# aehogan/lammps-induced-dipole-polarization-pair-style

Measured on AMD Instinct MI355X. Metric: atom-steps/sec, higher is better.
Workload: dtype f64

## Files before the change

### include/polar_mi355x.h

```cpp
#ifndef POLAR_MI355X_H
#define POLAR_MI355X_H

#ifdef __cplusplus
extern "C" {
#endif

#define POLAR_OK 0
#define POLAR_WARN_NOT_CONVERGED 1
#define POLAR_RETRY_STEP 2
#define POLAR_ERR_INPUT -1
#define POLAR_ERR_NO_DEVICE -2
#define POLAR_ERR_HIP -3
#define POLAR_ERR_UNSUPPORTED -4
#define POLAR_ERR_STATE -5

enum { POLAR_DAMP_EXPONENTIAL = 0, POLAR_DAMP_NONE = 1 };

typedef struct polar_handle polar_handle;

typedef struct {
  double cut_lj_global, cut_coul;
  double polar_precision, polar_damp, polar_gamma;
  int iterations_max, damping_type, zodid, fixed_iteration;
  int polar_gs, polar_gs_ranked, use_previous, debug;
// ... 80 lines not shown
                  polar_result *out);
int polar_compute_peratom(polar_handle *h, int eflag, int vflag, double *f, double *mu, double *ef_static,
                          double *eatom, double *vatom, polar_result *out);

int polar_get_debug_trace(polar_handle *h, double *u_polar, int max);

int polar_get_debug_forces(polar_handle *h, double *out6);

int polar_get_colors(polar_handle *h, int *color, int n);

int polar_set_colors(polar_handle *h, const int *color, int n);

int polar_compute_resident(polar_handle *h, int eflag, int vflag, polar_result *out);
void *polar_dev_ptr(polar_handle *h, const char *name);
int polar_download(polar_handle *h, const char *name, double *dst, long long n);
int polar_upload_mu(polar_handle *h, const double *mu, long long n);


int polar_set_stream(polar_handle *h, void *hip_stream);
int polar_set_row_range(polar_handle *h, int lo, int hi);
int polar_set_global_count(polar_handle *h, long long natoms);
int polar_set_list_style(polar_handle *h, int full);
int polar_step_begin(polar_handle *h, int eflag, int vflag);
int polar_step_sweep(polar_handle *h);
int polar_step_sweep_phase(polar_handle *h, int color, int part);
int polar_step_sweep_part(polar_handle *h, int part, int nparts);
int polar_step_sweep_end(polar_handle *h, const double *dev_global_change);
int polar_step_sweep_end_n(polar_handle *h, const double *dev_global_change, int count);
int polar_step_state(polar_handle *h, int *done, int *iterations, int *status);
int polar_step_finish(polar_handle *h, polar_result *out);
// ... 36 lines not shown
```

### lammps-induced-dipole-polarization-pair-style_amd/__init__.py

```python
from __future__ import annotations

import ctypes as C
import importlib
import os
import subprocess

import numpy as np

_HERE = os.path.dirname(os.path.abspath(__file__))
_CSRC = os.path.join(_HERE, "csrc")
LIB_PATH = os.path.join(_HERE, "libpolar_mi355x.so")
LIB_PATH_LAB = os.path.join(_HERE, "libpolar_mi355x_lab.so")
HIPCC = os.environ.get("HIPCC", "/opt/rocm/bin/hipcc")
HIP_FLAGS = ["--offload-arch=gfx950", "-O3", "-std=c++17", "-fPIC", "-shared"]

_lib = None
_lib_lab = None


class PolarError(RuntimeError):

    def __init__(self, code, message):
        super().__init__(message)
        self.code = code
# ... 82 lines not shown
    "polar_set_settings": (C.c_int, [C.c_void_p, C.POINTER(Settings)]),
    "polar_set_types": (C.c_int, [C.c_void_p, C.c_int] + [_dp] * 7),
    "polar_set_coul": (C.c_int, [C.c_void_p, C.c_double, C.c_double, _dp, _dp, C.c_int, C.c_int, C.c_int, C.c_double]
                       + [_dp] * 8),
    "polar_set_box": (C.c_int, [C.c_void_p, _dp, _dp, _dp, _ip, C.c_int]),
    "polar_set_atoms": (C.c_int, [C.c_void_p, C.c_int, C.c_int, _dp, _dp, _dp, _ip, _ip]),
    "polar_set_positions": (C.c_int, [C.c_void_p, C.c_int, C.c_int, _dp]),
    "polar_set_neighbors": (C.c_int, [C.c_void_p, C.c_int, _ip, _ip, C.POINTER(_ip)]),
    "polar_set_neighbors_csr": (C.c_int, [C.c_void_p, C.c_int, _ip, _ip, _llp, _ip]),
    "polar_build_neighbors": (C.c_int, [C.c_void_p, _dp, _ip, _ip, _ip, C.c_int, _ip, C.c_int]),
    "polar_compute": (C.c_int, [C.c_void_p, C.c_int, C.c_int, _dp, _dp, _dp, C.POINTER(Result)]),
    "polar_compute_peratom": (C.c_int, [C.c_void_p, C.c_int, C.c_int, _dp, _dp, _dp, _dp, _dp, C.POINTER(Result)]),
    "polar_compute_resident": (C.c_int, [C.c_void_p, C.c_int, C.c_int, C.POINTER(Result)]),
    "polar_dev_ptr": (C.c_void_p, [C.c_void_p, C.c_char_p]),
    "polar_download": (C.c_int, [C.c_void_p, C.c_char_p, _dp, C.c_longlong]),
    "polar_upload_mu": (C.c_int, [C.c_void_p, _dp, C.c_longlong]),
    "polar_set_stream": (C.c_int, [C.c_void_p, C.c_void_p]),
    "polar_set_row_range": (C.c_int, [C.c_void_p, C.c_int, C.c_int]),
    "polar_set_global_count": (C.c_int, [C.c_void_p, C.c_longlong]),
    "polar_step_mu_get": (C.c_int, [C.c_void_p, C.c_longlong, C.c_longlong, _dp]),
    "polar_step_mu_put_idx": (C.c_int, [C.c_void_p, C.c_longlong, _ip, _dp]),
    "polar_step_change_get": (C.c_int, [C.c_void_p, _dp]),
    "polar_step_sweep_end_host": (C.c_int, [C.c_void_p, C.c_double]),
    "polar_step_sweep_end_n": (C.c_int, [C.c_void_p, C.c_void_p, C.c_int]),
    "polar_set_list_style": (C.c_int, [C.c_void_p, C.c_int]),
    "polar_set_newton": (C.c_int, [C.c_void_p, C.c_int]),
    "polar_get_debug_trace": (C.c_int, [C.c_void_p, _dp, C.c_int]),
    "polar_get_debug_forces": (C.c_int, [C.c_void_p, _dp]),
    "polar_get_colors": (C.c_int, [C.c_void_p, C.POINTER(C.c_int), C.c_int]),
    "polar_restart_pack": (C.c_int, [C.c_void_p, C.c_void_p, C.c_int]),
# ... 313 lines not shown
    def debug_forces(self):
        a = np.zeros(6)
        self._ck(self.L.polar_get_debug_forces(self.h, _dptr(a)))
        return a[:3].copy(), a[3:].copy()

    def colors(self, n):
        a = np.full(n, -1, dtype=np.int32)
        nc = self._ck(self.L.polar_get_colors(self.h, a.ctypes.data_as(C.POINTER(C.c_int)), n))
        return nc, a

    def download(self, name, n):
        a = np.zeros(n)
        self._ck(self.L.polar_download(self.h, name.encode(), _dptr(a), n))
        return a


class PolarDist:

    @staticmethod
    def unique_id():
        buf = C.create_string_buffer(128)
        rc = lib().polar_dist_unique_id(buf)
        if rc < 0:
            raise PolarError(rc, "polar_dist_unique_id failed (is RCCL available?)")
        return buf.raw

    def __init__(self, unique_id, rank, nranks, device=0):
        self.L = lib()
        self.d = C.c_void_p()
        self.rank, self.nranks = rank, nranks
# ... 101 lines not shown
```

### lammps-induced-dipole-polarization-pair-style_amd/csrc/polar_api.hip

```cpp
#include "polar_handle.hpp"

namespace {
void upload_types(polar_handle *h, int ntypes, const double *const t[7]) {
  need_device(h);
  const size_t m = (size_t)(ntypes + 1) * (ntypes + 1);
  std::vector<double> pack(8 * m, 0.0);
  for (size_t k = 0; k < m; k++) {
    pack[8 * k + 0] = t[6][k]; pack[8 * k + 1] = t[5][k]; pack[8 * k + 2] = t[0][k]; pack[8 * k + 3] = t[1][k];
    pack[8 * k + 4] = t[2][k]; pack[8 * k + 5] = t[3][k]; pack[8 * k + 6] = t[4][k];
  }
  h->d_lj.ensure(8 * m);
  HIPCHECK(hipMemcpy(h->d_lj.p, pack.data(), 8 * m * sizeof(double), hipMemcpyHostToDevice));
  h->P.ntypes = ntypes;
  h->P.ljpack = h->d_lj.p;
  h->ntypes = ntypes;
  h->types_set = true;
}

void upload_coul(polar_handle *h, double g_ewald, double qqrd2e, const double *slj, const double *scoul, int nbits,
                 int mask, int shift, double tabinnersq, const double *const t[8]) {
  need_device(h);
  h->P.g_ewald = g_ewald; h->P.qqrd2e = qqrd2e;
  for (int k = 0; k < 4; k++) { h->P.special_lj[k] = slj[k]; h->P.special_coul[k] = scoul[k]; }
  h->P.ncoultablebits = nbits; h->P.ncoulmask = mask; h->P.ncoulshiftbits = shift; h->P.tabinnersq = tabinnersq;
// ... 123 lines not shown
int polar_device_count(void) {
  int n = 0;
  if (hipGetDeviceCount(&n) != hipSuccess) return 0;
  return n;
}

int polar_create(int device, polar_handle **out) {
  if (!out) return POLAR_ERR_STATE;
  polar_handle *h = new polar_handle();
  *out = h;
  h->device = device;
  if (const char *e = getenv("POLAR_COLOR_DIST")) h->color_dist = atof(e);
  h->color_keep = std::max(h->color_dist - 0.4, 0.75 * h->color_dist);
  if (const char *e = getenv("POLAR_COLOR_KEEP")) h->color_keep = atof(e);
  if (const char *e = getenv("POLAR_DETERMINISTIC")) h->deterministic = atoi(e) != 0;
#ifdef POLAR_LAB
#include "lab/api_env_knobs.inc"
#endif
  int n = polar_device_count();
  if (n <= 0 || device < 0 || device >= n) {
    h->have_device = false;
    h->err = "no usable HIP device";
    return POLAR_OK;
  }
  return guarded(h, [&]() {
    HIPCHECK(hipSetDevice(device));
    HIPCHECK(hipStreamCreate(&h->stream));
    for (auto &e : h->ev) HIPCHECK(hipEventCreate(&e));
    {
      int prio_lo = 0, prio_hi = 0;
// ... 37 lines not shown
    for (hipEvent_t e : h->ev_nl) (void)hipEventDestroy(e);
    for (hipEvent_t e : h->ev_fchunk) if (e) (void)hipEventDestroy(e);
    h->d_ljpos.release(); h->d_ljaux.release(); h->d_tag.release(); h->d_nspecial.release(); h->d_special.release();
    h->d_ljcell_id.release(); h->d_ljcell_cnt.release(); h->d_ljcell_fill.release(); h->d_ljcell_first.release(); h->d_cutneighsq.release();
    h->d_xchg.release(); h->d_xidx.release();
    h->d_eatom.release(); h->d_vatom.release(); h->d_dd_r2.release(); h->d_fpol.release();
    h->d_x.release(); h->d_q.release(); h->d_alpha.release(); h->d_f.release(); h->d_ef.release(); h->d_F.release();
    h->d_mu.release(); h->d_mu0.release(); h->d_acc_x.release(); h->d_acc_f.release(); h->d_acc_g.release(); h->d_acc_dF.release(); h->d_acc_dG.release(); h->d_acc_part.release(); h->d_acc_state.release(); h->d_bflag.release(); h->d_rank.release(); h->d_dmu.release(); h->d_tab.release(); h->d_lj.release();
    h->d_type.release(); h->d_mol.release(); h->d_order.release(); h->d_pos.release(); h->d_ilist.release();
    h->d_numneigh.release(); h->d_neigh.release(); h->d_rows.release(); h->d_first.release();
    h->d_sym_first.release(); h->d_sym_cnt.release(); h->d_sym_fill.release(); h->d_sym_j.release();
    h->d_mol_s.release(); h->d_perm.release(); h->d_inv.release(); h->d_rows_orig.release(); h->d_ownrows.release(); h->d_ef_s.release(); h->d_scan_a.release(); h->d_scan_b.release(); h->d_gs_cnt.release(); h->d_T6.release(); h->d_Minv.release(); h->d_gsN.release(); h->d_gsAT.release(); h->d_cb.release(); h->d_gs_part.release();
    h->d_rec0.release(); h->d_rec1.release(); h->d_scal.release(); h->d_slots.release();
    h->d_cell_id.release(); h->d_cell_cnt.release(); h->d_cell_fill.release();
    h->d_nl_cnt.release(); h->d_dd_cnt.release(); h->d_dd_wrap.release(); h->d_lpdesc.release(); h->d_slot.release(); h->d_color_orig.release(); h->d_color_s.release(); h->d_trace.release(); h->d_ew_kv.release(); h->d_ew_hkl.release(); h->d_ew_rows.release(); h->d_ew_s.release(); h->d_ew_m.release(); h->d_ew_part.release(); h->d_ew_erec.release(); h->d_ew_vpart.release(); h->d_ew_out.release(); h->d_cl_orig.release(); h->d_cl_cnt.release(); h->d_cl_wrap.release(); h->d_cl_tw.release(); h->d_cl_s.release(); h->d_nl_j.release(); h->d_dd_j.release();
    h->d_cell_first.release(); h->d_nl_first.release(); h->d_dd_first.release(); h->d_dd_s.release(); h->d_xq.release(); h->d_pos4.release();
    h->d_overflow.release(); h->d_ddtot.release();
    h->d_cadj.release(); h->d_cdeg.release(); h->d_ccnt.release(); h->d_cflags.release(); h->d_crelabel.release(); h->d_klist.release(); h->d_dbgf.release(); h->d_ulead.release(); h->d_udd_j.release(); h->d_upos.release(); h->d_unit.release(); h->d_udesc.release(); h->d_cprio.release(); h->d_cstat.release(); h->d_coff.release(); h->d_lp_pend.release(); h->d_lp_part.release();
    if (h->h_cflags) (void)hipHostFree(h->h_cflags);
    if (h->h_cstat) (void)hipHostFree(h->h_cstat);
    if (h->h_coff) (void)hipHostFree(h->h_coff);
    h->d_srec0.release(); h->d_srec1.release(); h->d_thdr.release(); h->d_trow.release(); h->d_un_j.release(); h->d_dd16.release(); h->d_pend.release();
    if (h->h_flags) (void)hipHostFree(h->h_flags);
    if (h->h_ddtot) (void)hipHostFree(h->h_ddtot);
    if (h->h_scal) (void)hipHostFree(h->h_scal);
    if (h->h_stage) (void)hipHostFree(h->h_stage);
    for (auto &e : h->ev) if (e) (void)hipEventDestroy(e);
    if (h->stream && h->own_stream) (void)hipStreamDestroy(h->stream);
  }
  delete h;
  return POLAR_OK;
// ... 474 lines not shown
    if (!out) throw std::runtime_error("polar_compute_resident: null result pointer");
    need_device(h);
    HIPCHECK(hipSetDevice(h->device));
    return do_compute(h, eflag, vflag, nullptr, out);
  });
}

void *polar_dev_ptr(polar_handle *h, const char *name) {
  if (!h || !name || !h->have_device) return nullptr;
  if (strcmp(name, "f") == 0) return h->d_f.p;
  if (strcmp(name, "mu") == 0) return h->d_mu.p;
  if (strcmp(name, "ef_static") == 0) return h->d_ef.p;
  if (strcmp(name, "x") == 0) return h->d_x.p;
  if (strcmp(name, "eatom") == 0) return h->d_eatom.p;
  if (strcmp(name, "vatom") == 0) return h->d_vatom.p;
  return nullptr;
}
int polar_download(polar_handle *h, const char *name, double *dst, long long n) {
  return guarded(h, [&]() {
    need_device(h);
    void *p = polar_dev_ptr(h, name);
    if (!p) throw std::runtime_error("polar_download: unknown array name");
    HIPCHECK(hipMemcpy(dst, p, (size_t)n * sizeof(double), hipMemcpyDeviceToHost));
    return POLAR_OK;
  });
}
int polar_upload_mu(polar_handle *h, const double *mu, long long n) {
  return guarded(h, [&]() {
    need_device(h);
    h->d_mu.ensure((size_t)n);
    HIPCHECK(hipMemcpy(h->d_mu.p, mu, (size_t)n * sizeof(double), hipMemcpyHostToDevice));
// ... 278 lines not shown
```

### lammps-induced-dipole-polarization-pair-style_amd/csrc/polar_handle.hpp

```cpp
#pragma once
#include <hip/hip_runtime.h>

#include <algorithm>
#include <initializer_list>
#include <utility>
#include <chrono>
#include <cmath>
#include <cstdio>
#include <cstdlib>
#include <exception>
#include <cstring>
#include <numeric>
#include <string>
#include <thread>
#include <mutex>
#include <condition_variable>
#include <functional>
#include <memory>
#include <stdexcept>
#include <unistd.h>
#include <vector>

#include "pair_host.hpp"
#include "polar_kernels.hpp"

using namespace polar;

#define POLAR_KERNEL_VERSION "r05-lp3-v3"
#define POLAR_MAX_CLASS_OFF 130


struct HipError : std::runtime_error {
  explicit HipError(const std::string &m) : std::runtime_error(m) {}
};
struct NoDevice : std::runtime_error {
  NoDevice() : std::runtime_error("no usable HIP device: this library has no CPU fallback") {}
};
#define HIPCHECK(expr)                                                                             \
  do {                                                                                             \
    hipError_t e_ = (expr);                                                                        \
    if (e_ != hipSuccess)                                                                          \
      throw HipError(std::string(#expr) + " failed: " + hipGetErrorString(e_) + " (" + __FILE__ + \
                     ":" + std::to_string(__LINE__) + ")");                                      \
// ... 98 lines not shown
  DBuf<double2> d_dd_s;
  DBuf<int2> d_lpdesc;
  DBuf<double> d_lp_pend;
  DBuf<double> d_lp_part;
  int lp_npart = 0;
  DBuf<int> d_slot;
  std::vector<int> h_cl;
  DBuf<int> d_cl_orig, d_cl_cnt, d_cl_wrap, d_cl_tw;
  DBuf<int4> d_cl_s;
  long long cl_pitch = 0;
  int ncl = 0;
  double cluster_dist = 2.0;
  int cluster_max = 4;
  long long cl_slots = 0;
  DBuf<double4> d_xq, d_pos4, d_xq_s;
  long long nl_pairs = 0, dd_pairs = 0;
  long long nl_pitch = 0, dd_pitch = 0;
  DBuf<int> d_overflow;
  DBuf<unsigned long long> d_ddtot;
  int *h_flags = nullptr;
  unsigned long long *h_ddtot = nullptr;
  int inum = 0;
  long long nneigh = 0;
  bool mu_resident = false;
  DBuf<double> d_dbgf;
  DBuf<double> d_acc_x, d_acc_f, d_acc_g, d_acc_dF, d_acc_dG, d_acc_part;
  DBuf<AccelState> d_acc_state;
  long long acc_pitch = 0; int acc_rows = 0;
  DBuf<double> d_mu0;
  bool mu0_saved = false;
// ... 82 lines not shown
  TileLaunch tile_all{};
  size_t tile_lds_attr[16] = {0, 0, 0, 0, 0, 0, 0, 0, 0, 0, 0, 0, 0, 0, 0, 0};
  size_t tile_build_lds_attr = 0;
  int tile_waves = 4;
  int tile_wide = 0;
  int tile_sw[3] = {2, 2, 2};
  int deterministic = 0;
  Scal *h_scal = nullptr;
  hipEvent_t ev[8] = {};
  hipStream_t lj_stream = nullptr;
  hipEvent_t ev_fork = nullptr, ev_join = nullptr, ev_lj0 = nullptr, ev_lj1 = nullptr, ev_dl0 = nullptr, ev_dl1 = nullptr;
  hipStream_t dl_stream = nullptr;
  hipEvent_t ev_mu_ready = nullptr;
  double *early_mu = nullptr, *early_ef = nullptr, *user_mu = nullptr, *user_ef = nullptr;
  hipEvent_t ev_fchunk[4] = {nullptr, nullptr, nullptr, nullptr};
  bool overlap_lj = true;
  bool lj_forked = false;
  std::vector<double> h_tmp;
  double *h_stage = nullptr;
  DBuf<double> d_trace;
  DBuf<double4> d_ew_kv; DBuf<int4> d_ew_hkl, d_ew_rows;
  DBuf<double2> d_ew_s, d_ew_m, d_ew_part;
  DBuf<double> d_ew_erec, d_ew_vpart, d_ew_out;
  std::vector<double> ew_key;
  int ew_nk = 0, ew_nrow = 0, ew_nm = 0;
  double ew_cell[6] = {0, 0, 0, 0, 0, 0};
  hipEvent_t ev_ks[4] = {nullptr, nullptr, nullptr, nullptr};
  int ntrace = 0;
  size_t h_stage_cap = 0;
};
// ... 188 lines not shown
```

### lammps-induced-dipole-polarization-pair-style_amd/csrc/polar_lists.hpp

```cpp
#pragma once

#include "polar_common.hpp"

namespace polar {

struct CellGrid {
  int trim;
  int nc[3];
  double lo[3], inv[3];
};

__device__ __forceinline__ int cell_of(const CellGrid &g, const Box &b, double x, double y, double z) {
  int c[3];
  double fr3[3];
  frac_coords(b, g.lo, x, y, z, fr3);
#pragma unroll
  for (int k = 0; k < 3; k++) {
    double fr = fr3[k];
    fr -= floor(fr);
    int ck = (int)(fr * g.nc[k]);
    c[k] = ck >= g.nc[k] ? g.nc[k] - 1 : ck;
  }
  return (c[2] * g.nc[1] + c[1]) * g.nc[0] + c[0];
}
// ... 543 lines not shown
          if (RECHECK && icol >= 0 && rsq < colordistsq && __double2loint(rj.w) && color_s[j] == icol) clash = true;
          wrap_lane |= in_dd && shifted;
          same = (imol != 0 && imol == __double2hiint(rj.w)) ? POLAR_NL_SAMEMOL : 0;
        }
        const unsigned long long m_nl = __ballot(in_nl), m_dd = __ballot(in_dd);
        const int kn = ncount + __popcll(m_nl & below), kd = dcount + __popcll(m_dd & below);
        if (in_nl && kn < nl_pitch) nl_j[nl0 + kn] = j | same;
        if (in_dd && kd < dd_pitch) {
          dd_j[dd0 + (dd_shift ? lp_slot(kd, dd_qm) : (long long)kd)] = j << dd_shift;
          if (dd_r2) dd_r2[dd0 + kd] = rsq;
        }
        ncount += __popcll(m_nl);
        dcount += __popcll(m_dd);
      }
    }
  }
  if (pad_dd) {
    const int have = dcount < dd_pitch ? dcount : (int)dd_pitch;
    const int padded = (have + 63) & ~63;
    for (int k = have + lane; k < padded; k += 64) {
      dd_j[dd0 + (dd_shift ? lp_slot(k, dd_qm) : (long long)k)] = (dd_pad_index >= 0 ? dd_pad_index : i) << dd_shift;
      if (dd_r2) dd_r2[dd0 + k] = 1e60;
    }
  }
  if (RECHECK && color_s && __ballot(clash) != 0ull && lane == 0) atomicOr(color_conflict, 1);
  const unsigned long long anywrap = __ballot(wrap_lane);
  if (lane == 0) {
    nl_cnt[i] = ncount; dd_cnt[i] = dcount;
    if (dd_wrap) dd_wrap[i] = anywrap != 0ull;
    if (ncount > nl_pitch || dcount > dd_pitch) atomicMax(overflow, ncount > dcount ? ncount : dcount);
// ... 252 lines not shown
```

### lammps-induced-dipole-polarization-pair-style_amd/csrc/polar_rows.hpp

```cpp
#pragma once

#include "polar_common.hpp"

namespace polar {

static __global__ void k_pack(int n, const int *__restrict__ perm, const double *__restrict__ x, const double *__restrict__ q,
                       const double *__restrict__ alpha, const int *__restrict__ mol, const double *__restrict__ mu0,
                       AtomRec *__restrict__ r0, AtomRec *__restrict__ r1, int *__restrict__ mol_s,
                       double4 *__restrict__ pos4, double4 *__restrict__ xq_s, int wrap, Box box, double lo0, double lo1,
                       double lo2) {
  int i = blockIdx.x * blockDim.x + threadIdx.x;
  if (i == n) {
    AtomRec d;
    d.x = n > 0 ? x[0] : 0.0; d.y = n > 0 ? x[1] : 0.0; d.z = n > 0 ? x[2] : 0.0;
    d.mx = d.my = d.mz = d.q = d.a = 0.0;
    r0[n] = d; r1[n] = d;
  }
  if (i >= n) return;
  const int o = perm ? perm[i] : i;
  AtomRec r;
  r.x = x[3 * o]; r.y = x[3 * o + 1]; r.z = x[3 * o + 2]; r.q = q[o];
  if (wrap) {
    const double lo[3] = {lo0, lo1, lo2};
    double fr[3];
    frac_coords(box, lo, r.x, r.y, r.z, fr);
    const double n2 = box.periodic[2] ? floor(fr[2]) : 0.0, n1 = box.periodic[1] ? floor(fr[1]) : 0.0,
                 n0 = box.periodic[0] ? floor(fr[0]) : 0.0;
    r.z -= n2 * box.prd[2]; r.y -= n2 * box.yz + n1 * box.prd[1]; r.x -= n2 * box.xz + n1 * box.xy + n0 * box.prd[0];
  }
  r.mx = mu0 ? mu0[3 * o] : 0.0; r.my = mu0 ? mu0[3 * o + 1] : 0.0; r.mz = mu0 ? mu0[3 * o + 2] : 0.0;
  r.a = alpha[o];
  r0[i] = r;
  r1[i] = r;
  mol_s[i] = mol[o];
  if (pos4) pos4[i] = make_double4(r.x, r.y, r.z, __hiloint2double(mol[o], r.a != 0.0 ? 1 : 0));
  if (xq_s) xq_s[i] = make_double4(r.x, r.y, r.z, r.q);
}

template <bool ALLPAIRS, int PASS>
static __global__ __launch_bounds__(POLAR_BLOCK) void k_rank(int nlocal, int ntotal, const double *__restrict__ x,
                                                      const double *__restrict__ alpha, const int *__restrict__ mol,
                                                      Box box, RowList nl,
                                                      const int *__restrict__ nl_j,
                                                      const AtomRec *__restrict__ rec,
                                                      const int *__restrict__ mol_s, Scal *scal,
                                                      double *__restrict__ slots,
                                                      double *__restrict__ rank_metric, int nchunk) {
  const int lane = threadIdx.x & 63;
  const int gw = blockIdx.x * POLAR_ROWS_PER_BLOCK + (threadIdx.x >> 6);
  if (gw >= nlocal * nchunk) return;
  const int i = gw % nlocal, chunk = gw / nlocal;
// ... 614 lines not shown
```

### lammps-induced-dipole-polarization-pair-style_amd/csrc/polar_step.hip

```cpp
#include "polar_handle.hpp"

void launch_scan(long long n, const int *in, long long *out, DBuf<long long> &tot, hipStream_t s) {
  const int nb = (int)std::max<long long>(1, (n + POLAR_SCAN_ITEMS - 1) / POLAR_SCAN_ITEMS);
  tot.ensure((size_t)nb + 1);
  k_scan_block<<<nb, 1024, 0, s>>>(n, in, out, tot.p);
  if (nb > 1) {
    k_scan_totals<<<1, 1024, 0, s>>>(nb, tot.p, out + n);
    k_scan_add<<<nblk(n - POLAR_SCAN_ITEMS, 256), 256, 0, s>>>(n, out, tot.p);
  }
}

void build_cells(polar_handle *h) {
  const polar_settings &st = h->ph.st;
  const int n = h->nlocal;
  const double cutall = std::max(st.cut_coul, st.dd_cutoff);
  double width[3];
  box_widths(h->box, width);
  for (int k = 0; k < 3; k++)
    if (h->box.periodic[k] && width[k] < 2.0 * cutall * (1.0 - 1e-12))
      throw InputError("dd_cutoff mode needs box lengths >= 2*max(cut_coul,dd_cutoff); use exact mode (dd_cutoff 0)");
  CellGrid &g = h->grid;
  g.trim = 1;
#ifdef POLAR_LAB
  if (const char *e = getenv("POLAR_NL_TRIM")) g.trim = atoi(e);
// ... 23 lines not shown
    }
    h->tile_launches.clear();
    for (const Cls &cz : cls[2]) for (const Cls &cy : cls[1]) for (const Cls &cx : cls[0]) {
      TileLaunch L;
      L.start[0] = cx.start; L.stride[0] = cx.stride; L.count[0] = cx.count;
      L.start[1] = cy.start; L.stride[1] = cy.stride; L.count[1] = cy.count;
      L.start[2] = cz.start; L.stride[2] = cz.stride; L.count[2] = cz.count;
      for (int k = 0; k < 3; k++) L.nc[k] = g.nc[k];
      h->tile_launches.push_back(L);
    }
    for (int k = 0; k < 3; k++) { h->tile_all.start[k] = 0; h->tile_all.stride[k] = 1; h->tile_all.count[k] = g.nc[k]; h->tile_all.nc[k] = g.nc[k]; }
  }
  hipStream_t s = h->stream;
  h->d_cell_id.ensure(n); h->d_cell_cnt.ensure(ncell + 1); h->d_cell_fill.ensure(2 * (ncell + 1));
  h->d_cell_first.ensure(ncell + 2); h->d_perm.ensure(n + 1); h->d_inv.ensure(n + 1);
  zero_many(s, {{h->d_cell_cnt.p, (size_t)(ncell + 1) * sizeof(int)}, {h->d_cell_fill.p, 2 * (size_t)(ncell + 1) * sizeof(int)}});
  k_cell_count<<<nblk(n, 256), 256, 0, s>>>(n, h->d_x.p, g, h->box, h->d_cell_id.p, h->d_cell_cnt.p);
  launch_scan(ncell, h->d_cell_cnt.p, h->d_cell_first.p, h->d_scan_a, s);
  k_cell_fill<<<nblk(n, 256), 256, 0, s>>>(n, h->d_cell_id.p, h->d_cell_first.p, h->d_cell_fill.p,
                                           (h->pol_first || h->sweep_kernel == 4) ? h->d_cell_fill.p + ncell + 1 : nullptr, h->d_alpha.p, h->d_perm.p, h->d_inv.p);
  k_cell_sort<<<nblk(ncell, 4), 256, 0, s>>>(ncell, h->d_cell_first.p, (h->pol_first || h->sweep_kernel == 4) ? h->d_cell_fill.p : nullptr, h->d_perm.p, h->d_inv.p);
  h->sorted = true;
  if (sharded(h)) {
    h->d_ownrows.ensure(own_n(h) + 1);
    k_map_range<<<nblk(own_n(h), 256), 256, 0, s>>>(own_lo(h), own_n(h), h->d_inv.p, h->d_ownrows.p);
  }
}

void compute_slots(polar_handle *h) {
  const polar_settings &st = h->ph.st;
  const bool gs = st.polar_gs || st.polar_gs_ranked;
// ... 70 lines not shown
  if (getenv("POLAR_NO_FUSE_R2")) fuse = false;
#endif
  const double cutallsq = cutall * cutall, ddsq = mode == 4 ? -1.0 : st.dd_cutoff * st.dd_cutoff;
  const int nr = own_n(h);
  const int *rows = own_rows(h);
  zero_many(s, {{h->d_nl_cnt.p, (size_t)(n + 1) * sizeof(int)}, {h->d_dd_cnt.p, (size_t)(n + 1) * sizeof(int)},
                {h->d_overflow.p, 16 * sizeof(int)}, {h->d_ddtot.p, 64 * 16 * sizeof(unsigned long long)}});
  const bool lp = mode == 3;
  if (lp) h->d_dd_wrap.ensure(n + 1);
  const bool recheck = h->colors_valid && h->colors_recheck && h->sweep_kernel < 3 && (int)h->h_color.size() == n;
  if (h->colors_recheck && !recheck) { h->colors_valid = false; h->colors_recheck = false; }
  if (recheck) {
    h->d_color_s.ensure(n + 1);
    k_color_map<<<nblk(n, 256), 256, 0, s>>>(n, h->d_perm.p, h->d_color_orig.p, h->d_color_s.p);
  }
#define NLB(TRI, RC)                                                                                                          \
  k_nl_build<TRI, RC><<<nblk(nr, POLAR_ROWS_PER_BLOCK), POLAR_BLOCK, 0, s>>>(                                                 \
      rows, nr, h->d_pos4.p, h->box, g, h->d_cell_first.p, cutallsq, ddsq, h->nl_pitch, h->dd_pitch, h->d_nl_cnt.p,            \
      h->d_dd_cnt.p, h->d_nl_j.p, h->d_dd_j.p, fuse ? r2p : nullptr, fuse ? 1 : 0, lp ? (6 | (h->lp_quad_major << 8)) : 0,    \
      lp ? n : -1, lp ? h->d_dd_wrap.p : nullptr, recheck ? h->d_color_s.p : nullptr, h->color_keep * h->color_keep,           \
      h->d_overflow.p + 8, lp ? h->d_slot.p : nullptr, h->d_overflow.p, h->d_ddtot.p)
  if (h->box.triclinic) { if (recheck) NLB(true, true); else NLB(true, false); }
  else                  { if (recheck) NLB(false, true); else NLB(false, false); }
#undef NLB
  const RowList ddl{h->d_dd_cnt.p, h->dd_pitch};
  if (fuse || mode == 4) {
  }
#ifdef POLAR_LAB
  else if (st.damping_type == POLAR_DAMP_EXPONENTIAL)
    k_dd_scalars<0><<<nblk(nr, POLAR_ROWS_PER_BLOCK), POLAR_BLOCK, 0, s>>>(rows, nr, h->d_rec0.p, h->box, ddl, h->d_dd_j.p, st.polar_damp, sp, r2p);
  else
    k_dd_scalars<1><<<nblk(nr, POLAR_ROWS_PER_BLOCK), POLAR_BLOCK, 0, s>>>(rows, nr, h->d_rec0.p, h->box, ddl, h->d_dd_j.p, st.polar_damp, sp, r2p);
#endif
  HIPCHECK(hipMemcpyAsync(h->h_flags, h->d_overflow.p, sizeof(int), hipMemcpyDeviceToHost, s));
  HIPCHECK(hipMemcpyAsync(h->h_ddtot, h->d_ddtot.p, 64 * 16 * sizeof(unsigned long long), hipMemcpyDeviceToHost, s));
}
template <bool AP>
static void launch_rank(polar_handle *h, int pass) {
  const int n = h->nlocal, ntot = h->nlocal + h->nghost;
// ... 634 lines not shown
  h->sorted = false;
  h->dense_gs = false;
  const bool gs_mode = (st.polar_gs || st.polar_gs_ranked) && !st.zodid;
  bool ranked_done = false;
  if (ap && gs_mode && n > 64 && 48.0 * (double)n * (double)n <= 3.2e10 && !getenv("POLAR_NO_DENSE_GS")) {
    h->dense_gs = true;
    if (st.polar_gs_ranked) {
      launch_rank<true>(h, 1); launch_rank<true>(h, 2);
      ranked_done = true;
      h->d_perm.ensure(n + 1); h->d_inv.ensure(n + 1);
      k_rank_order<<<nblk(n, POLAR_ROWS_PER_BLOCK), POLAR_BLOCK, 0, s>>>(n, h->d_rank.p, h->d_perm.p, h->d_inv.p);
      h->sorted = true;
    }
  }
  if (!ap) { build_cells(h); h->d_pos4.ensure(n + 1); if (h->static_xq) h->d_xq_s.ensure(n + 2); }
  k_pack<<<nblk(n + 1, 256), 256, 0, s>>>(n, h->sorted ? h->d_perm.p : nullptr, h->d_x.p, h->d_q.p, h->d_alpha.p, h->d_mol.p, mu0,
                                      h->d_rec0.p, h->d_rec1.p, h->d_mol_s.p, ap ? nullptr : h->d_pos4.p, (!ap && h->static_xq) ? h->d_xq_s.p : nullptr,
                                      (!ap && h->sweep_kernel == 4) ? 1 : 0, h->box, h->boxlo[0], h->boxlo[1], h->boxlo[2]);
  if (!ap) {
    if (h->colors_valid && h->sweep_kernel < 3) map_color_rows(h);
    if (h->sweep_kernel == 2) compute_slots(h);
    build_lists(h);
    if (h->colors_valid && h->sweep_kernel == 3) build_cluster_lists(h);
    if (h->sweep_kernel == 4) build_tiles(h);
  }
  HIPCHECK(hipEventRecord(h->ev[1], s));

  if (st.polar_gs_ranked && (ap || (!h->colors_valid && h->sweep_kernel != 4)) && !ranked_done) {
    if (ap) { launch_rank<true>(h, 1); launch_rank<true>(h, 2); }
    else    { launch_rank<false>(h, 1); launch_rank<false>(h, 2); }
  }
  HIPCHECK(hipEventRecord(h->ev[2], s));

// ... 205 lines not shown
```

Before: 15.57 million.

## Add packed neighbor-list build with per-run shifted images and lazy min-image

```diff
diff --git a/include/polar_mi355x.h b/include/polar_mi355x.h
--- a/include/polar_mi355x.h
+++ b/include/polar_mi355x.h
@@ -118,6 +118,7 @@
 int polar_compute_resident(polar_handle *h, int eflag, int vflag, polar_result *out);
 void *polar_dev_ptr(polar_handle *h, const char *name);
 int polar_download(polar_handle *h, const char *name, double *dst, long long n);
+int polar_list_shape(polar_handle *h, long long *out);
 int polar_upload_mu(polar_handle *h, const double *mu, long long n);
 
 
diff --git a/lammps-induced-dipole-polarization-pair-style_amd/__init__.py b/lammps-induced-dipole-polarization-pair-style_amd/__init__.py
--- a/lammps-induced-dipole-polarization-pair-style_amd/__init__.py
+++ b/lammps-induced-dipole-polarization-pair-style_amd/__init__.py
@@ -120,6 +120,7 @@
     "polar_compute_resident": (C.c_int, [C.c_void_p, C.c_int, C.c_int, C.POINTER(Result)]),
     "polar_dev_ptr": (C.c_void_p, [C.c_void_p, C.c_char_p]),
     "polar_download": (C.c_int, [C.c_void_p, C.c_char_p, _dp, C.c_longlong]),
+    "polar_list_shape": (C.c_int, [C.c_void_p, _llp]),
     "polar_upload_mu": (C.c_int, [C.c_void_p, _dp, C.c_longlong]),
     "polar_set_stream": (C.c_int, [C.c_void_p, C.c_void_p]),
     "polar_set_row_range": (C.c_int, [C.c_void_p, C.c_int, C.c_int]),
@@ -463,6 +464,27 @@
         self._ck(self.L.polar_download(self.h, name.encode(), _dptr(a), n))
         return a
 
+    def lists(self):
+        sh = np.zeros(8, dtype=np.int64)
+        self._ck(self.L.polar_list_shape(self.h, sh.ctypes.data_as(_llp)))
+        n, nlp, ddp, mode = (int(v) for v in sh[:4])
+
+        def ints(name, count):
+            return self.download(name, (count + 1) // 2).view(np.int32)[:count].copy()
+
+        out = {"nl_pitch": nlp, "dd_pitch": ddp, "mode": mode, "flags": ints("list_flags", 16)}
+        for k in ("perm", "nl_cnt", "dd_cnt"):
+            out[k] = ints(k, n)
+        out["nl_j"] = ints("nl_j", n * nlp).reshape(n, nlp)
+        if sh[5] >= n * ddp:
+            out["dd_j"] = ints("dd_j", n * ddp).reshape(n, ddp)
+        if mode == 1 and sh[6] >= n * ddp:
+            out["dd_r2"] = self.download("dd_r2", n * ddp).reshape(n, ddp)
+        if mode == 3 and sh[7] >= n:
+            out["dd_wrap"] = ints("dd_wrap", n)
+            out["dd_slot"] = ints("dd_slot", n)
+        return out
+
 
 class PolarDist:
 
diff --git a/lammps-induced-dipole-polarization-pair-style_amd/csrc/polar_api.hip b/lammps-induced-dipole-polarization-pair-style_amd/csrc/polar_api.hip
--- a/lammps-induced-dipole-polarization-pair-style_amd/csrc/polar_api.hip
+++ b/lammps-induced-dipole-polarization-pair-style_amd/csrc/polar_api.hip
@@ -161,6 +161,7 @@
   h->color_keep = std::max(h->color_dist - 0.4, 0.75 * h->color_dist);
   if (const char *e = getenv("POLAR_COLOR_KEEP")) h->color_keep = atof(e);
   if (const char *e = getenv("POLAR_DETERMINISTIC")) h->deterministic = atoi(e) != 0;
+  if (const char *e = getenv("POLAR_NL_PACK")) h->nl_pack = atoi(e) != 0;
 #ifdef POLAR_LAB
 #include "lab/api_env_knobs.inc"
 #endif
@@ -228,7 +229,7 @@
     h->d_rec0.release(); h->d_rec1.release(); h->d_scal.release(); h->d_slots.release();
     h->d_cell_id.release(); h->d_cell_cnt.release(); h->d_cell_fill.release();
     h->d_nl_cnt.release(); h->d_dd_cnt.release(); h->d_dd_wrap.release(); h->d_lpdesc.release(); h->d_slot.release(); h->d_color_orig.release(); h->d_color_s.release(); h->d_trace.release(); h->d_ew_kv.release(); h->d_ew_hkl.release(); h->d_ew_rows.release(); h->d_ew_s.release(); h->d_ew_m.release(); h->d_ew_part.release(); h->d_ew_erec.release(); h->d_ew_vpart.release(); h->d_ew_out.release(); h->d_cl_orig.release(); h->d_cl_cnt.release(); h->d_cl_wrap.release(); h->d_cl_tw.release(); h->d_cl_s.release(); h->d_nl_j.release(); h->d_dd_j.release();
-    h->d_cell_first.release(); h->d_nl_first.release(); h->d_dd_first.release(); h->d_dd_s.release(); h->d_xq.release(); h->d_pos4.release();
+    h->d_cell_first.release(); h->d_nl_first.release(); h->d_dd_first.release(); h->d_dd_s.release(); h->d_xq.release(); h->d_pos4.release(); h->d_pos4w.release(); h->d_nl_far.release();
     h->d_overflow.release(); h->d_ddtot.release();
     h->d_cadj.release(); h->d_cdeg.release(); h->d_ccnt.release(); h->d_cflags.release(); h->d_crelabel.release(); h->d_klist.release(); h->d_dbgf.release(); h->d_ulead.release(); h->d_udd_j.release(); h->d_upos.release(); h->d_unit.release(); h->d_udesc.release(); h->d_cprio.release(); h->d_cstat.release(); h->d_coff.release(); h->d_lp_pend.release(); h->d_lp_part.release();
     if (h->h_cflags) (void)hipHostFree(h->h_cflags);
@@ -733,7 +734,22 @@
   if (strcmp(name, "x") == 0) return h->d_x.p;
   if (strcmp(name, "eatom") == 0) return h->d_eatom.p;
   if (strcmp(name, "vatom") == 0) return h->d_vatom.p;
+  if (strcmp(name, "perm") == 0) return h->d_perm.p;
+  if (strcmp(name, "nl_cnt") == 0) return h->d_nl_cnt.p;
+  if (strcmp(name, "dd_cnt") == 0) return h->d_dd_cnt.p;
+  if (strcmp(name, "nl_j") == 0) return h->d_nl_j.p;
+  if (strcmp(name, "dd_j") == 0) return h->d_dd_j.p;
+  if (strcmp(name, "dd_r2") == 0) return h->d_dd_r2.p;
+  if (strcmp(name, "dd_wrap") == 0) return h->d_dd_wrap.p;
+  if (strcmp(name, "dd_slot") == 0) return h->d_slot.p;
+  if (strcmp(name, "list_flags") == 0) return h->d_overflow.p;
   return nullptr;
+}
+int polar_list_shape(polar_handle *h, long long *out) {
+  if (!h || !out) return POLAR_ERR_STATE;
+  out[0] = h->nlocal; out[1] = h->nl_pitch; out[2] = h->dd_pitch; out[3] = h->stream_mode;
+  out[4] = (long long)h->d_nl_j.cap; out[5] = (long long)h->d_dd_j.cap; out[6] = (long long)h->d_dd_r2.cap; out[7] = (long long)h->d_dd_wrap.cap;
+  return POLAR_OK;
 }
 int polar_download(polar_handle *h, const char *name, double *dst, long long n) {
   return guarded(h, [&]() {
diff --git a/lammps-induced-dipole-polarization-pair-style_amd/csrc/polar_handle.hpp b/lammps-induced-dipole-polarization-pair-style_amd/csrc/polar_handle.hpp
--- a/lammps-induced-dipole-polarization-pair-style_amd/csrc/polar_handle.hpp
+++ b/lammps-induced-dipole-polarization-pair-style_amd/csrc/polar_handle.hpp
@@ -26,7 +26,7 @@
 
 using namespace polar;
 
-#define POLAR_KERNEL_VERSION "r05-lp3-v3"
+#define POLAR_KERNEL_VERSION "r06-nlpk-v1"
 #define POLAR_MAX_CLASS_OFF 130
 
 
@@ -155,6 +155,8 @@
   int cluster_max = 4;
   long long cl_slots = 0;
   DBuf<double4> d_xq, d_pos4, d_xq_s;
+  DBuf<double4> d_pos4w;
+  DBuf<int> d_nl_far;
   long long nl_pairs = 0, dd_pairs = 0;
   long long nl_pitch = 0, dd_pitch = 0;
   DBuf<int> d_overflow;
@@ -267,6 +269,7 @@
   hipEvent_t ev_mu_ready = nullptr;
   double *early_mu = nullptr, *early_ef = nullptr, *user_mu = nullptr, *user_ef = nullptr;
   hipEvent_t ev_fchunk[4] = {nullptr, nullptr, nullptr, nullptr};
+  bool nl_pack = true;
   bool overlap_lj = true;
   bool lj_forked = false;
   std::vector<double> h_tmp;
diff --git a/lammps-induced-dipole-polarization-pair-style_amd/csrc/polar_lists.hpp b/lammps-induced-dipole-polarization-pair-style_amd/csrc/polar_lists.hpp
--- a/lammps-induced-dipole-polarization-pair-style_amd/csrc/polar_lists.hpp
+++ b/lammps-induced-dipole-polarization-pair-style_amd/csrc/polar_lists.hpp
@@ -581,6 +581,207 @@
         dcount += __popcll(m_dd);
       }
     }
+  }
+  if (pad_dd) {
+    const int have = dcount < dd_pitch ? dcount : (int)dd_pitch;
+    const int padded = (have + 63) & ~63;
+    for (int k = have + lane; k < padded; k += 64) {
+      dd_j[dd0 + (dd_shift ? lp_slot(k, dd_qm) : (long long)k)] = (dd_pad_index >= 0 ? dd_pad_index : i) << dd_shift;
+      if (dd_r2) dd_r2[dd0 + k] = 1e60;
+    }
+  }
+  if (RECHECK && color_s && __ballot(clash) != 0ull && lane == 0) atomicOr(color_conflict, 1);
+  const unsigned long long anywrap = __ballot(wrap_lane);
+  if (lane == 0) {
+    nl_cnt[i] = ncount; dd_cnt[i] = dcount;
+    if (dd_wrap) dd_wrap[i] = anywrap != 0ull;
+    if (ncount > nl_pitch || dcount > dd_pitch) atomicMax(overflow, ncount > dcount ? ncount : dcount);
+    if (dcount) atomicAdd(dd_total + (blockIdx.x & 63) * 16, (unsigned long long)(dcount < dd_pitch ? dcount : (int)dd_pitch));
+  }
+}
+
+struct alignas(16) NlRun {
+  double x, y, z;
+  int off, key;
+};
+template <bool TRI, bool RECHECK, bool SHIFT>
+static __global__ __launch_bounds__(POLAR_BLOCK) void k_nl_build_pk(const int *__restrict__ rows, int nrows,
+                                                             const double4 *__restrict__ pos4,
+                                                             const double4 *__restrict__ pos4w, const int *__restrict__ far,
+                                                             double win_abs, Box box, CellGrid g,
+                                                             const long long *__restrict__ cell_first, double cutallsq,
+                                                             double ddcutsq, long long nl_pitch, long long dd_pitch,
+                                                             int *__restrict__ nl_cnt, int *__restrict__ dd_cnt,
+                                                             int *__restrict__ nl_j, int *__restrict__ dd_j,
+                                                             double *__restrict__ dd_r2, int pad_dd,
+                                                             int dd_shift_qm, int dd_pad_index, int *__restrict__ dd_wrap,
+                                                             const int *__restrict__ color_s, double colordistsq,
+                                                             int *__restrict__ color_conflict,
+                                                             const int *__restrict__ dd_slot,
+                                                             int *__restrict__ overflow,
+                                                             unsigned long long *__restrict__ dd_total) {
+  __shared__ NlRun tab_all[POLAR_ROWS_PER_BLOCK][64];
+  const int dd_shift = dd_shift_qm & 255, dd_qm = dd_shift_qm >> 8;
+  const int lane = threadIdx.x & 63;
+  const int row = blockIdx.x * POLAR_ROWS_PER_BLOCK + (threadIdx.x >> 6);
+  if (row >= nrows) return;
+  NlRun *tab = tab_all[threadIdx.x >> 6];
+  const int i = rows ? rows[row] : row;
+  const double4 ri = pos4[i];
+  const int imol = __double2hiint(ri.w), ipol = __double2loint(ri.w);
+  const int icol = (RECHECK && color_s && ipol) ? color_s[i] : -2;
+  bool clash = RECHECK && color_s && ipol && icol < 0;
+  int cc[3];
+  double uu[3], edge[3];
+  {
+    double fr3[3];
+    frac_coords(box, g.lo, ri.x, ri.y, ri.z, fr3);
+#pragma unroll
+    for (int k = 0; k < 3; k++) {
+      double fr = fr3[k];
+      fr -= floor(fr);
+      const double t = fr * g.nc[k];
+      int ck = (int)t;
+      ck = ck >= g.nc[k] ? g.nc[k] - 1 : ck;
+      cc[k] = __builtin_amdgcn_readfirstlane(ck);
+      uu[k] = wave_uniform(t - ck); edge[k] = wave_uniform(box.prd[k] / g.nc[k]);
+    }
+  }
+  const int c0 = cc[0], c1 = cc[1], c2 = cc[2];
+  const int slot_i = dd_slot ? dd_slot[i] : i;
+  const long long nl0 = (long long)i * nl_pitch, dd0 = (long long)(slot_i >= 0 ? slot_i : 0) * dd_pitch;
+  int ncount = 0, dcount = 0;
+  bool wrap_lane = false;
+  const unsigned long long below = (lane == 0) ? 0ull : (~0ull >> (64 - lane));
+  const int n0 = g.nc[0], n1 = g.nc[1], n2 = g.nc[2];
+  const int zlo = n2 >= 5 ? c2 - 2 : 0, zcnt = n2 >= 5 ? 5 : n2;
+  const int ylo = n1 >= 5 ? c1 - 2 : 0, ycnt = n1 >= 5 ? 5 : n1;
+  const double reach = sqrt(cutallsq > ddcutsq ? cutallsq : ddcutsq) + 1e-6;
+  const double reach2 = wave_uniform(reach * reach);
+  const int nsr = zcnt * ycnt;
+  int ra0 = 0, rb0 = 0, ra1 = 0, rb1 = 0;
+  int sx = 0, sy = 0, sz = 0;
+  if (lane < nsr) {
+    const int zz = zlo + lane / ycnt, yy = ylo + lane % ycnt;
+    int b2 = zz, b1 = yy;
+    bool ok = true;
+    if (b2 < 0 || b2 >= n2) { if (!box.periodic[2]) ok = false; b2 = (b2 + n2) % n2; sz = zz < 0 ? -1 : 1; }
+    if (b1 < 0 || b1 >= n1) { if (!box.periodic[1]) ok = false; b1 = (b1 + n1) % n1; sy = yy < 0 ? -1 : 1; }
+    double dzmin = 0.0, dymin = 0.0;
+    if (n2 >= 5) { const int d = zz - c2; dzmin = d > 0 ? (d - uu[2]) * edge[2] : (d < 0 ? (uu[2] - (d + 1)) * edge[2] : 0.0); }
+    if (n1 >= 5) { const int d = yy - c1; dymin = d > 0 ? (d - uu[1]) * edge[1] : (d < 0 ? (uu[1] - (d + 1)) * edge[1] : 0.0); }
+    const double rem2 = reach2 - dzmin * dzmin - dymin * dymin;
+    if (g.trim && rem2 < 0.0) ok = false;
+    int xlo = n0 >= 5 ? c0 - 2 : 0, xhi = n0 >= 5 ? c0 + 2 : n0 - 1;
+    if (ok && g.trim && n0 >= 5) {
+      const double xr = sqrt(rem2) / edge[0];
+      int lo_off = (int)floor(uu[0] - xr), hi_off = (int)floor(uu[0] + xr);
+      lo_off = lo_off < -2 ? -2 : lo_off; hi_off = hi_off > 2 ? 2 : hi_off;
+      xlo = c0 + lo_off; xhi = c0 + hi_off;
+    }
+    if (ok) {
+      const long long rowbase = ((long long)b2 * n1 + b1) * n0;
+      const int xa = xlo < 0 ? 0 : xlo, xb = xhi >= n0 ? n0 - 1 : xhi;
+      ra0 = (int)cell_first[rowbase + xa]; rb0 = (int)cell_first[rowbase + xb + 1];
+      if (box.periodic[0]) {
+        if (xlo < 0) { ra1 = (int)cell_first[rowbase + xlo + n0]; rb1 = (int)cell_first[rowbase + n0]; sx = -1; }
+        else if (xhi >= n0) { ra1 = (int)cell_first[rowbase]; rb1 = (int)cell_first[rowbase + xhi - n0 + 1]; sx = 1; }
+      }
+    }
+  }
+  const int len0 = rb0 - ra0, len1 = rb1 - ra1;
+  int incl = len0 + len1;
+#pragma unroll
+  for (int d = 1; d < 64; d <<= 1) {
+    const int u = __shfl_up(incl, d);
+    if (lane >= d) incl += u;
+  }
+  const int total = __builtin_amdgcn_readlane(incl, 63);
+  const int start0 = incl - len0 - len1, start1 = start0 + len0;
+  if (lane < 32) {
+    NlRun r0, r1;
+    r0.off = ra0 - start0; r1.off = ra1 - start1;
+    r0.x = r0.y = r0.z = r1.x = r1.y = r1.z = 0.0;
+    r0.key = r1.key = 0;
+    if (SHIFT) {
+      const double4 wi = pos4w[i];
+      const int code = __double2loint(wi.w) >> 1;
+      const int fx = code & 1023, fy = (code >> 10) & 1023, fz = (code >> 20) & 1023;
+      r0.y = r1.y = wi.y - sy * box.prd[1];
+      r0.z = r1.z = wi.z - sz * box.prd[2];
+      r0.x = wi.x;
+      r1.x = wi.x - sx * box.prd[0];
+      const int kyz = (((fy + sy) & 1023) << 10) | (((fz + sz) & 1023) << 20);
+      r0.key = kyz | fx;
+      r1.key = kyz | ((fx + sx) & 1023);
+    }
+    tab[2 * lane] = r0; tab[2 * lane + 1] = r1;
+  }
+  const int rs0 = __shfl(start0, lane >> 1), rs1 = __shfl(start1, lane >> 1);
+  const int rs = (lane & 1) ? rs1 : rs0;
+  __builtin_amdgcn_fence(__ATOMIC_RELEASE, "wavefront");
+  __builtin_amdgcn_wave_barrier();
+  __builtin_amdgcn_fence(__ATOMIC_ACQUIRE, "wavefront");
+  const bool exact_all = SHIFT && (far[0] != 0 || dd_r2 != nullptr);
+  const double win_nl = 1e-12 * cutallsq + sqrt(cutallsq) * win_abs;
+  const double win_dd = ddcutsq > 0.0 ? 1e-12 * ddcutsq + sqrt(ddcutsq) * win_abs : 0.0;
+  const double win_col = colordistsq > 0.0 ? 1e-12 * colordistsq + sqrt(colordistsq) * win_abs : 0.0;
+  for (int base = 0; base < total; base += 64) {
+    const int v = base + lane;
+    int r = __popcll(__ballot(rs <= base)) - 1;
+    unsigned long long inside = __ballot(rs > base && rs < total && rs < base + 64);
+    while (inside) {
+      const int q = __builtin_ctzll(inside);
+      inside &= inside - 1;
+      r += v >= __builtin_amdgcn_readlane(rs, q) ? 1 : 0;
+    }
+    const NlRun R = tab[r];
+    const int p = v + R.off;
+    bool in_nl = false, in_dd = false;
+    const int j = p;
+    int same = 0;
+    double rsq = 0.0;
+    if (v < total && j != i) {
+      bool shifted;
+      int wj;
+      if (SHIFT) {
+        const double4 rj = pos4w[j];
+        const double ex = R.x - rj.x, ey = R.y - rj.y, ez = R.z - rj.z;
+        rsq = ex * ex + ey * ey + ez * ez;
+        wj = __double2loint(rj.w);
+        shifted = (wj >> 1) != R.key;
+        same = (imol != 0 && imol == __double2hiint(rj.w)) ? POLAR_NL_SAMEMOL : 0;
+        const bool near = exact_all || fabs(rsq - cutallsq) <= win_nl || fabs(rsq - ddcutsq) <= win_dd ||
+                          (RECHECK && icol >= 0 && fabs(rsq - colordistsq) <= win_col);
+        if (near) {
+          const double4 ro = pos4[j];
+          double fx, fy, fz;
+          shifted = min_image_rint_w<false>(box, ri.x, ri.y, ri.z, ro.x, ro.y, ro.z, fx, fy, fz);
+          rsq = fx * fx + fy * fy + fz * fz;
+        }
+        wj &= 1;
+      } else {
+        const double4 rj = pos4[j];
+        double ex, ey, ez;
+        shifted = min_image_rint_w<TRI>(box, ri.x, ri.y, ri.z, rj.x, rj.y, rj.z, ex, ey, ez);
+        rsq = ex * ex + ey * ey + ez * ez;
+        wj = __double2loint(rj.w);
+        same = (imol != 0 && imol == __double2hiint(rj.w)) ? POLAR_NL_SAMEMOL : 0;
+      }
+      in_nl = rsq <= cutallsq;
+      in_dd = ipol && slot_i >= 0 && wj && (rsq < ddcutsq);
+      if (RECHECK && icol >= 0 && rsq < colordistsq && wj && color_s[j] == icol) clash = true;
+      wrap_lane |= in_dd && shifted;
+    }
+    const unsigned long long m_nl = __ballot(in_nl), m_dd = __ballot(in_dd);
+    const int kn = ncount + __popcll(m_nl & below), kd = dcount + __popcll(m_dd & below);
+    if (in_nl && kn < nl_pitch) nl_j[nl0 + kn] = j | same;
+    if (in_dd && kd < dd_pitch) {
+      dd_j[dd0 + (dd_shift ? lp_slot(kd, dd_qm) : (long long)kd)] = j << dd_shift;
+      if (dd_r2) dd_r2[dd0 + kd] = rsq;
+    }
+    ncount += __popcll(m_nl);
+    dcount += __popcll(m_dd);
   }
   if (pad_dd) {
     const int have = dcount < dd_pitch ? dcount : (int)dd_pitch;
diff --git a/lammps-induced-dipole-polarization-pair-style_amd/csrc/polar_rows.hpp b/lammps-induced-dipole-polarization-pair-style_amd/csrc/polar_rows.hpp
--- a/lammps-induced-dipole-polarization-pair-style_amd/csrc/polar_rows.hpp
+++ b/lammps-induced-dipole-polarization-pair-style_amd/csrc/polar_rows.hpp
@@ -8,7 +8,7 @@
                        const double *__restrict__ alpha, const int *__restrict__ mol, const double *__restrict__ mu0,
                        AtomRec *__restrict__ r0, AtomRec *__restrict__ r1, int *__restrict__ mol_s,
                        double4 *__restrict__ pos4, double4 *__restrict__ xq_s, int wrap, Box box, double lo0, double lo1,
-                       double lo2) {
+                       double lo2, double4 *__restrict__ pos4w, int *__restrict__ nl_far) {
   int i = blockIdx.x * blockDim.x + threadIdx.x;
   if (i == n) {
     AtomRec d;
@@ -35,6 +35,22 @@
   mol_s[i] = mol[o];
   if (pos4) pos4[i] = make_double4(r.x, r.y, r.z, __hiloint2double(mol[o], r.a != 0.0 ? 1 : 0));
   if (xq_s) xq_s[i] = make_double4(r.x, r.y, r.z, r.q);
+  if (pos4w) {
+    const double lo[3] = {lo0, lo1, lo2};
+    double p[3] = {x[3 * o], x[3 * o + 1], x[3 * o + 2]}, fr[3];
+    frac_coords(box, lo, p[0], p[1], p[2], fr);
+    int code = 0;
+    bool out = false;
+#pragma unroll
+    for (int k = 0; k < 3; k++) {
+      const double w = box.periodic[k] ? floor(fr[k]) : 0.0;
+      p[k] -= w * box.prd[k];
+      out |= w < -1.0 || w > 1.0;
+      code |= ((int)fmax(-512.0, fmin(511.0, w)) & 1023) << (10 * k);
+    }
+    pos4w[i] = make_double4(p[0], p[1], p[2], __hiloint2double(mol[o], (code << 1) | (r.a != 0.0 ? 1 : 0)));
+    if (out) atomicOr(nl_far, 1);
+  }
 }
 
 template <bool ALLPAIRS, int PASS>
diff --git a/lammps-induced-dipole-polarization-pair-style_amd/csrc/polar_step.hip b/lammps-induced-dipole-polarization-pair-style_amd/csrc/polar_step.hip
--- a/lammps-induced-dipole-polarization-pair-style_amd/csrc/polar_step.hip
+++ b/lammps-induced-dipole-polarization-pair-style_amd/csrc/polar_step.hip
@@ -8,6 +8,13 @@
     k_scan_totals<<<1, 1024, 0, s>>>(nb, tot.p, out + n);
     k_scan_add<<<nblk(n - POLAR_SCAN_ITEMS, 256), 256, 0, s>>>(n, out, tot.p);
   }
+}
+
+static bool nl_shift(const polar_handle *h) {
+  if (!h->nl_pack || h->box.triclinic) return false;
+  for (int k = 0; k < 3; k++)
+    if (h->box.periodic[k] && h->grid.nc[k] < 6) return false;
+  return true;
 }
 
 void build_cells(polar_handle *h) {
@@ -61,7 +68,9 @@
   hipStream_t s = h->stream;
   h->d_cell_id.ensure(n); h->d_cell_cnt.ensure(ncell + 1); h->d_cell_fill.ensure(2 * (ncell + 1));
   h->d_cell_first.ensure(ncell + 2); h->d_perm.ensure(n + 1); h->d_inv.ensure(n + 1);
-  zero_many(s, {{h->d_cell_cnt.p, (size_t)(ncell + 1) * sizeof(int)}, {h->d_cell_fill.p, 2 * (size_t)(ncell + 1) * sizeof(int)}});
+  h->d_nl_far.ensure(1);
+  zero_many(s, {{h->d_cell_cnt.p, (size_t)(ncell + 1) * sizeof(int)}, {h->d_cell_fill.p, 2 * (size_t)(ncell + 1) * sizeof(int)},
+                {h->d_nl_far.p, sizeof(int)}});
   k_cell_count<<<nblk(n, 256), 256, 0, s>>>(n, h->d_x.p, g, h->box, h->d_cell_id.p, h->d_cell_cnt.p);
   launch_scan(ncell, h->d_cell_cnt.p, h->d_cell_first.p, h->d_scan_a, s);
   k_cell_fill<<<nblk(n, 256), 256, 0, s>>>(n, h->d_cell_id.p, h->d_cell_first.p, h->d_cell_fill.p,
@@ -162,15 +171,31 @@
     h->d_color_s.ensure(n + 1);
     k_color_map<<<nblk(n, 256), 256, 0, s>>>(n, h->d_perm.p, h->d_color_orig.p, h->d_color_s.p);
   }
-#define NLB(TRI, RC)                                                                                                          \
-  k_nl_build<TRI, RC><<<nblk(nr, POLAR_ROWS_PER_BLOCK), POLAR_BLOCK, 0, s>>>(                                                 \
-      rows, nr, h->d_pos4.p, h->box, g, h->d_cell_first.p, cutallsq, ddsq, h->nl_pitch, h->dd_pitch, h->d_nl_cnt.p,            \
+#define NLB_ARGS                                                                                                              \
+      h->box, g, h->d_cell_first.p, cutallsq, ddsq, h->nl_pitch, h->dd_pitch, h->d_nl_cnt.p,                                   \
       h->d_dd_cnt.p, h->d_nl_j.p, h->d_dd_j.p, fuse ? r2p : nullptr, fuse ? 1 : 0, lp ? (6 | (h->lp_quad_major << 8)) : 0,    \
       lp ? n : -1, lp ? h->d_dd_wrap.p : nullptr, recheck ? h->d_color_s.p : nullptr, h->color_keep * h->color_keep,           \
-      h->d_overflow.p + 8, lp ? h->d_slot.p : nullptr, h->d_overflow.p, h->d_ddtot.p)
-  if (h->box.triclinic) { if (recheck) NLB(true, true); else NLB(true, false); }
-  else                  { if (recheck) NLB(false, true); else NLB(false, false); }
+      h->d_overflow.p + 8, lp ? h->d_slot.p : nullptr, h->d_overflow.p, h->d_ddtot.p
+#define NLB(TRI, RC) k_nl_build<TRI, RC><<<nblk(nr, POLAR_ROWS_PER_BLOCK), POLAR_BLOCK, 0, s>>>(rows, nr, h->d_pos4.p, NLB_ARGS)
+#define NLP(TRI, RC, SH)                                                                                                      \
+  k_nl_build_pk<TRI, RC, SH><<<nblk(nr, POLAR_ROWS_PER_BLOCK), POLAR_BLOCK, 0, s>>>(rows, nr, h->d_pos4.p, h->d_pos4w.p,       \
+                                                                                  h->d_nl_far.p, win_abs, NLB_ARGS)
+  if (!h->nl_pack) {
+    if (h->box.triclinic) { if (recheck) NLB(true, true); else NLB(true, false); }
+    else                  { if (recheck) NLB(false, true); else NLB(false, false); }
+  } else {
+    const bool shift = nl_shift(h) && !(fuse && r2p);
+    double win_abs = 0.0;
+    for (int k = 0; k < 3; k++)
+      if (h->box.periodic[k]) win_abs = std::max(win_abs, std::fabs(h->boxlo[k]) + 3.0 * h->box.prd[k]);
+    win_abs *= std::ldexp(1.0, -47);
+    if (h->box.triclinic) { if (recheck) NLP(true, true, false); else NLP(true, false, false); }
+    else if (shift)       { if (recheck) NLP(false, true, true); else NLP(false, false, true); }
+    else                  { if (recheck) NLP(false, true, false); else NLP(false, false, false); }
+  }
+#undef NLP
 #undef NLB
+#undef NLB_ARGS
   const RowList ddl{h->d_dd_cnt.p, h->dd_pitch};
   if (fuse || mode == 4) {
   }
@@ -835,9 +860,12 @@
     }
   }
   if (!ap) { build_cells(h); h->d_pos4.ensure(n + 1); if (h->static_xq) h->d_xq_s.ensure(n + 2); }
+  const bool pos4w = !ap && nl_shift(h);
+  if (pos4w) h->d_pos4w.ensure(n + 1);
   k_pack<<<nblk(n + 1, 256), 256, 0, s>>>(n, h->sorted ? h->d_perm.p : nullptr, h->d_x.p, h->d_q.p, h->d_alpha.p, h->d_mol.p, mu0,
                                       h->d_rec0.p, h->d_rec1.p, h->d_mol_s.p, ap ? nullptr : h->d_pos4.p, (!ap && h->static_xq) ? h->d_xq_s.p : nullptr,
-                                      (!ap && h->sweep_kernel == 4) ? 1 : 0, h->box, h->boxlo[0], h->boxlo[1], h->boxlo[2]);
+                                      (!ap && h->sweep_kernel == 4) ? 1 : 0, h->box, h->boxlo[0], h->boxlo[1], h->boxlo[2],
+                                      pos4w ? h->d_pos4w.p : nullptr, h->d_nl_far.p);
   if (!ap) {
     if (h->colors_valid && h->sweep_kernel < 3) map_color_rows(h);
     if (h->sweep_kernel == 2) compute_slots(h);
```

Result: no change. 15.72 million (median of 6 runs) (+1.0%).
